# pvangoor/eqvio

Measured on AMD Instinct MI355X. Metric: EqF vision updates/sec @ N=200 landmarks, higher is better.
Workload: dtype f64; 1 GPU; synthetic 'hover' world, 200 tracked landmarks (state dim 621, 400 measurement rows), InvDepth chart, fast Riccati, IMU 200 Hz / camera 20 Hz (10 observer steps per frame), EuRoC pinhole intrinsics, one independent filter per GPU (replicas); landmarks=200, state_dim=621, parallelism=replicas x1

## Files before the change

eqvio_amd/capi.py:

```python
import ctypes as C
import os

import numpy as np

_HERE = os.path.dirname(os.path.abspath(__file__))
LIB_DIR = os.environ.get("EQVIO_AMD_LIB_DIR") or os.path.join(_HERE, "lib")

COORD_EUCLIDEAN, COORD_INVDEPTH, COORD_NORMAL = 0, 1, 2
OPT_RICCATI_DENSE, OPT_CHECK_FINITE, OPT_SIGMA_FP32, OPT_DOORBELL, OPT_SPECULATIVE, OPT_EARLY_LIFT, OPT_TRACE, OPT_FUSED_ASSEMBLY, OPT_LOOKAHEAD, OPT_LA_TIMEOUT_US, OPT_Z_IN_LOOKAHEAD, OPT_LA_SPLIT_ROWS, OPT_MEASURE_IN_PROPAGATE, OPT_LIFT_WITH_SYRK, OPT_LA_HOME, OPT_TILES_PER_WORKGROUP, OPT_GATHER_IN_PROPAGATE, OPT_HOLD_NEW_LANDMARKS, OPT_SELECT_ONE_WORKGROUP, OPT_LIVE_COLUMNS_FIRST, OPT_EARLY_DOORBELL, OPT_QUIET_DOOR_WAIT, OPT_INNOVATION_STATS, OPT_TIMING = 1, 2, 3, 6, 7, 8, 9, 11, 12, 15, 17, 18, 19, 20, 21, 22, 23, 24, 25, 26, 27, 29, 30, 100

c_double_p = C.POINTER(C.c_double)
c_int_p = C.POINTER(C.c_int)


class Camera(C.Structure):

    _fields_ = [
        ("model", C.c_int),
        ("width", C.c_int),
        ("height", C.c_int),
        ("fx", C.c_double),
        ("fy", C.c_double),
        ("cx", C.c_double),
        ("cy", C.c_double),
        ("dist", C.c_double * 5),
    ]

    @staticmethod
    def pinhole(fx, fy, cx, cy, width, height):
        cam = Camera()
        cam.model, cam.width, cam.height = 0, int(width), int(height)
        cam.fx, cam.fy, cam.cx, cam.cy = fx, fy, cx, cy
        return cam

    @staticmethod
    def radtan(fx, fy, cx, cy, width, height, k1, k2, p1, p2, k3=0.0):
        cam = Camera.pinhole(fx, fy, cx, cy, width, height)
        cam.model = 1
        cam.dist[:] = [k1, k2, p1, p2, k3]
        return cam

    @staticmethod
# ... 141 lines not shown
        "eqf_add_landmarks_held": (C.c_int, [vp, c_int_p, c_double_p, C.c_int, C.c_double]),
        "eqf_hold_supported": (C.c_int, [vp]),
        "eqf_hold_stats": (C.c_int, [vp, C.POINTER(C.c_long), C.c_int]),
        "eqf_live_columns_stats": (C.c_int, [vp, C.POINTER(C.c_long), C.c_int]),
        "eqf_own_hardware_queue": (C.c_int, [vp]),
        "eqf_remove_invalid_landmarks": (C.c_int, [vp]),
        "eqf_integrate_riccati_fast": (C.c_int, [vp, c_double_p, C.c_double, c_double_p, c_double_p]),
        "eqf_integrate_riccati_accurate": (C.c_int, [vp, c_double_p, C.c_double, c_double_p, c_double_p]),
        "eqf_integrate_riccati_discrete": (C.c_int, [vp, c_double_p, C.c_double, c_double_p, c_double_p]),
        "eqf_integrate_observer": (C.c_int, [vp, c_double_p, c_double_p, C.c_int, C.c_int]),
        "eqf_outlier_stats": (C.c_int, [vp, P(Camera), c_int_p, c_double_p, C.c_int, c_double_p, c_double_p, c_double_p]),
        "eqf_propagate_fast": (C.c_int, [vp, c_double_p, C.c_double, c_double_p, c_double_p, c_double_p, c_double_p, C.c_int, C.c_int]),
        "eqf_stage_measurement": (C.c_int, [vp, c_int_p, c_double_p, C.c_int]),
        "eqf_trace_read": (C.c_int, [vp, C.POINTER(C.c_ulonglong), C.POINTER(C.c_longlong), C.POINTER(C.c_uint)]),
        "eqf_host_wait_stats": (C.c_int, [vp, C.POINTER(C.c_long), c_double_p, C.c_int]),
        "eqf_stats_then_update": (C.c_int, [vp, C.POINTER(Camera), c_int_p, c_double_p, C.c_int, C.c_double, C.c_double, C.c_double, C.c_int, C.c_int, c_double_p, c_double_p,
                                  c_double_p, c_int_p]),
        "eqf_stats_select_update": (C.c_int, [vp, C.POINTER(Camera), c_int_p, c_double_p, C.c_int, C.c_double, C.c_double, C.c_int, C.c_double, C.c_int, C.c_int, c_double_p,
                                    c_double_p, c_double_p, c_int_p, c_int_p, c_int_p]),
        "eqf_vision_update": (C.c_int, [vp, P(Camera), c_int_p, c_double_p, C.c_int, C.c_double, C.c_int, C.c_int]),
        "eqf_last_gamma": (C.c_int, [vp, c_double_p, C.c_int]),
        "eqf_compute_nees": (C.c_int, [vp, c_double_p, c_int_p, c_double_p, C.c_int, c_double_p]),
        "eqf_nees_lu_fallbacks": (C.c_int, [vp, C.POINTER(C.c_long)]),
        "eqf_speculation_stats": (C.c_int, [vp, C.POINTER(C.c_long), C.POINTER(C.c_long), C.POINTER(C.c_long), C.c_int]),
        "eqf_measure_in_propagate_stats": (C.c_int, [vp, C.POINTER(C.c_long), C.c_int]),
        "eqf_z_in_lookahead_stats": (C.c_int, [vp, C.POINTER(C.c_long), C.c_int]),
        "eqf_gather_stats": (C.c_int, [vp, C.POINTER(C.c_long), C.c_int]),
        "eqf_selection_stats": (C.c_int, [vp, C.POINTER(C.c_long), C.POINTER(C.c_long), C.c_int]),
        "eqf_output_cov_all": (C.c_int, [vp, P(Camera), c_double_p]),
        "eqf_lookahead_stats": (C.c_int, [vp, C.POINTER(C.c_long), C.POINTER(C.c_long), C.c_int]),
        "eqf_debug_matrices_AB": (C.c_int, [vp, c_double_p, c_double_p, c_double_p]),
        "eqf_debug_get_W": (C.c_int, [vp, c_double_p, C.c_int, C.c_int]),
        "eqf_debug_syrk_order": (C.c_int, [C.c_int, c_int_p]),
        "eqf_debug_lookahead_stamps": (C.c_int, [vp, C.POINTER(C.c_ulonglong)]),
        "eqf_debug_matrix_C": (C.c_int, [vp, P(Camera), c_int_p, c_double_p, C.c_int, C.c_int, c_double_p, c_double_p]),
        "eqf_mfma_f64_peak": (C.c_int, [vp, c_double_p]),
        "eqf_mfma_f64_peak_clock": (C.c_int, [vp, C.POINTER(C.c_double), C.POINTER(C.c_double)]),
        "eqf_last_kernel_times": (C.c_int, [vp, c_int_p, P(C.c_float), C.c_int]),
        "eqf_last_innovation": (C.c_int, [vp, c_int_p, c_double_p, c_double_p]),
        "eqf_innovation_totals": (C.c_int, [vp, P(C.c_long), P(C.c_long), c_double_p, c_double_p]),
        "eqf_reset_innovation_totals": (C.c_int, [vp]),
    }
    for name, (res, args) in protos.items():
        if os.environ.get("EQVIO_AMD_LIB_DIR") and name in ("eqf_lookahead_home", "eqf_device_to_itself", "eqf_early_doorbell_stats", "eqf_update_unsettled", "eqf_remove_invalid_at_update", "eqf_gather_stats", "eqf_remove_unmeasured_landmarks", "eqf_find_unknown_ids", "eqf_add_landmarks_held", "eqf_hold_supported", "eqf_hold_stats", "eqf_same_as_mapped", "eqf_live_columns_stats", "eqf_own_hardware_queue", "eqf_last_innovation", "eqf_innovation_totals", "eqf_reset_innovation_totals") and not hasattr(lib, name):
            continue
        fn = getattr(lib, name)
        fn.restype = res
        fn.argtypes = args
    lib._declared = sorted(protos)
    _lib = lib
    return lib


class EqfCore:

    def __init__(self, max_landmarks, coordinate_choice=COORD_EUCLIDEAN, device=0):
        self.lib = load_eqf_lib()
        self.h = C.c_void_p()
        self._chk0(self.lib.eqf_create(C.byref(self.h), device, max_landmarks, coordinate_choice))
        self._cap0 = max_landmarks + 16

    def _chk0(self, rc):
        if rc != 0:
            raise EqfError(rc, self.lib.eqf_error_string(rc).decode())

    def close(self):
        if self.h:
            self.lib.eqf_destroy(self.h)
            self.h = C.c_void_p()

    def __del__(self):
        try:
            self.close()
        except Exception:
            pass

    @property
# ... 557 lines not shown
```

eqvio_amd/csrc/eqf_hip.hip:

```cpp
#include "eqf_hip.h"
#include "eqf_kernels.hpp"
#include "eqf_lookahead.hpp"
#include "eqf_innovation.hpp"
#include "eqf_batch.hpp"
#include "eqf_batch.h"
#include "host_prof.hpp"
#include <algorithm>
#include <atomic>
#include <chrono>
#include <condition_variable>
#include <deque>
#include <limits>
#include <mutex>
#include <optional>
#include <cstdio>
#include <cstdlib>
#include <cstring>
#include <string>
#include <vector>
#include <unistd.h>
#include <fcntl.h>
#include <signal.h>
#include <sys/mman.h>
#include <cerrno>
// ... 69 lines not shown
    g.bacc = v3(s[3], s[4], s[5]);
    g.A = Pose{Qt{s[6], s[7], s[8], s[9]}, v3(s[10], s[11], s[12])};
    g.w = v3(s[13], s[14], s[15]);
    g.B = Pose{Qt{s[16], s[17], s[18], s[19]}, v3(s[20], s[21], s[22])};
    return g;
}
void pack_group(const GroupSensor& g, double* s) {
    pack_v3(g.bgyr, s);
    pack_v3(g.bacc, s + 3);
    pack_pose(g.A, s + 6, s + 10);
    pack_v3(g.w, s + 13);
    pack_pose(g.B, s + 16, s + 20);
}

}

struct TailPlan {
    int M = 0, m = 0, n = 0, rows = 0;
    double meas_var = 0.0;
    int discreteCorr = 0;
    const int* spec = nullptr;
    int spec_seq = 0;
    bool use_door = false;
    int door_seq = 0;
    MeasFuse mf{};
    const int* live_cols = nullptr;
    bool ident = false;
    bool la = false;
    bool chain_only = false;
    int zb = 0;
    bool build_z = false;
    bool in_prop = false;
    bool lift_with_syrk = false;
    bool lift_before_syrk = false;
    bool syrk_gamma = false;
    int early_seq = 0;
    bool sig32 = false, check = false;
    bool innov = false;
    bool masked = false;
};


struct CtxOptions {
    int opt_dense = 0, opt_check = 0, opt_timing = 0, opt_f32 = 0, opt_early = 1, opt_fuse_asm = 1;
    int opt_door = 1;
    int opt_spec = 1;
    int opt_la_home = 1;
    int opt_lookahead = 1;
    int opt_zb = 1;
    int opt_zb_large = 1;
    int opt_la_split = 1;
    int opt_prop_tpw = 1;
    int opt_gather = 1;
    int opt_early_door = 1;
    int opt_quiet_wait = 1;
    int opt_la_watch_ahead = 1;
    int opt_hold = 1;
    int opt_sel_one = 1;
    int opt_live_first = 1;
    int opt_measure_prop = 1;
    int opt_lift_syrk = 1;
    int opt_innov = 0;
    long long la_timeout_ticks = LA_TIMEOUT_TICKS;
};
struct CtxCounters {
    long la_launches = 0, la_fallbacks = 0;
    int la_consecutive_stalls = 0;
    long la_home_launches = 0;
    long la_home_refused = 0;
    long la_book_timeouts = 0;
    long zb_launches = 0;
    long early_rings = 0;
    long live_first_launches = 0;
    long held_launches = 0;
    long gather_launches = 0;
    long me_used = 0;
    int spec_backoff = 0, spec_backoff_len = 0;
    long spec_calls = 0, spec_queued = 0, spec_cancelled = 0;
    long sel_frames = 0, sel_discarded = 0;
    long nees_lu_fallbacks = 0;
    long wait_calls = 0, launch_calls = 0;
    double wait_seconds = 0.0, launch_seconds = 0.0;
    long innov_updates = 0, innov_dof = 0;
    double innov_nis = 0.0, innov_logdet = 0.0;
    int innov_last_kind = 0;
    int innov_last_dof = 0;
    double innov_last_nis = 0.0, innov_last_logdet = 0.0;
};
enum { INNOV_NONE = 0, INNOV_VALUE, INNOV_FAILED, INNOV_OFF };
struct InnovPending {
    int kind, slot, seq, m;
};
struct CtxBuffers {
    std::vector<void*> device, pinned;
};

struct eqf_ctx : CtxOptions, CtxCounters {
    CtxBuffers own;
    int device = 0;
    hipStream_t stream = nullptr;
    hipStream_t stream2 = nullptr;
    hipEvent_t ev_assembled = nullptr, ev_observer = nullptr, ev_early = nullptr;
    bool ev_assembled_early = false;
    bool obs_pending = false;
    bool busy_common = false, busy_steps = false, busy_meas = false;
    int chart = 0;
    int Ncap = 0, ncap = 0, ld = 0;
    int mcap = 0, ldz = 0;
    int N = 0;
// ... 840 lines not shown
    return 0;
}

enum OptKind { OPT_PLAIN, OPT_BOOL , OPT_RANGE  };
struct OptRow {
    int id;
    int CtxOptions::*member;
    OptKind kind;
    int lo, hi;
};
static const OptRow kOptions[] = {
    {EQF_OPT_RICCATI_DENSE, &CtxOptions::opt_dense, OPT_PLAIN, 0, 0},
    {EQF_OPT_CHECK_FINITE, &CtxOptions::opt_check, OPT_PLAIN, 0, 0},
    {EQF_OPT_SIGMA_FP32, &CtxOptions::opt_f32, OPT_RANGE, 0, 3},
    {EQF_OPT_SPECULATIVE, &CtxOptions::opt_spec, OPT_PLAIN, 0, 0},
    {EQF_OPT_DOORBELL, &CtxOptions::opt_door, OPT_PLAIN, 0, 0},
    {EQF_OPT_EARLY_LIFT, &CtxOptions::opt_early, OPT_PLAIN, 0, 0},
    {EQF_OPT_FUSED_ASSEMBLY, &CtxOptions::opt_fuse_asm, OPT_PLAIN, 0, 0},
    {EQF_OPT_LOOKAHEAD, &CtxOptions::opt_lookahead, OPT_PLAIN, 0, 0},
    {EQF_OPT_LA_TIMEOUT_US, nullptr, OPT_RANGE, 0, INT_MAX},
    {EQF_OPT_Z_IN_LOOKAHEAD, nullptr, OPT_PLAIN, 0, 0},
    {EQF_OPT_LA_SPLIT_ROWS, &CtxOptions::opt_la_split, OPT_BOOL, 0, 0},
    {EQF_OPT_LA_HOME, &CtxOptions::opt_la_home, OPT_PLAIN, 0, 0},
    {EQF_OPT_TILES_PER_WORKGROUP, &CtxOptions::opt_prop_tpw, OPT_RANGE, 0, 8},
    {EQF_OPT_GATHER_IN_PROPAGATE, &CtxOptions::opt_gather, OPT_BOOL, 0, 0},
    {EQF_OPT_HOLD_NEW_LANDMARKS, &CtxOptions::opt_hold, OPT_BOOL, 0, 0},
    {EQF_OPT_SELECT_ONE_WORKGROUP, &CtxOptions::opt_sel_one, OPT_BOOL, 0, 0},
    {EQF_OPT_LIVE_COLUMNS_FIRST, &CtxOptions::opt_live_first, OPT_BOOL, 0, 0},
    {EQF_OPT_EARLY_DOORBELL, &CtxOptions::opt_early_door, OPT_BOOL, 0, 0},
    {EQF_OPT_QUIET_DOOR_WAIT, &CtxOptions::opt_quiet_wait, OPT_BOOL, 0, 0},
    {EQF_OPT_MEASURE_IN_PROPAGATE, &CtxOptions::opt_measure_prop, OPT_BOOL, 0, 0},
    {EQF_OPT_LIFT_WITH_SYRK, &CtxOptions::opt_lift_syrk, OPT_BOOL, 0, 0},
    {EQF_OPT_INNOVATION_STATS, &CtxOptions::opt_innov, OPT_BOOL, 0, 0},
    {EQF_OPT_TRACE, nullptr, OPT_PLAIN, 0, 0},
    {100, &CtxOptions::opt_timing, OPT_PLAIN, 0, 0},
    {102, &CtxOptions::opt_la_watch_ahead, OPT_BOOL, 0, 0},
};
static const OptRow* option_row(int option) {
    for (const OptRow& r : kOptions)
        if (r.id == option)
            return &r;
    return nullptr;
}

int eqf_get_option(const eqf_ctx* c, int option, int* value) {
    const OptRow* row = c && value ? option_row(option) : nullptr;
    if (!row)
        return EQF_E_BAD_ARG;
    if (row->member)
        *value = c->*(row->member);
    else if (option == EQF_OPT_Z_IN_LOOKAHEAD)
        *value = c->opt_zb ? (c->opt_zb_large ? 1 : 2) : 0;
    else if (option == EQF_OPT_LA_TIMEOUT_US)
        *value = (int)(c->la_timeout_ticks / 100);
    else
        *value = c->d_trace ? 1 : 0;
    return 0;
}
int eqf_set_option(eqf_ctx* c, int option, int value) {
    const OptRow* row = c ? option_row(option) : nullptr;
    if (!row)
        return EQF_E_BAD_ARG;
    if (row->kind == OPT_BOOL)
        value = value ? 1 : 0;
    else if (row->kind == OPT_RANGE && (value < row->lo || value > row->hi))
        return EQF_E_BAD_ARG;
// ... 1545 lines not shown
    c->la_home_force = true;
    int rc = lookahead_selftest_pass(c, refused);
    c->la_home_force = false;
    if (rc)
        return rc;
    const bool home_on = c->opt_la_home != 0;
    if (home_on && (refused || c->la_selftest < 0)) {
        std::fprintf(stderr, "[eqf_hip] device %d: the look-ahead kernel's HOME placement %s; this context uses the classic placement\n", c->device,
                     refused ? "was refused (blocks are not dealt to the XCDs round robin)" : "failed its self-test");
        c->opt_la_home = 0;
        c->la_selftest = 0;
        rc = lookahead_selftest_pass(c, refused);
        if (rc)
            return rc;
    }
    if (c->la_selftest < 0)
        std::fprintf(stderr, "[eqf_hip] look-ahead self-test failed on device %d: this context factorises on the launch chain\n", c->device);
    c->la_home_launches = 0;
    return 0;
}
static bool tail_use_door(const eqf_ctx* c) { return c->opt_door && !c->opt_check && !c->obs_pending; }
struct TailCall {
    const int* ids;
    int M;
    double meas_var;
    int discreteCorr;
    bool use_door;
    int door_seq;
    const MeasFuse* fuse = nullptr;
    bool live_first = false;
    bool takes_early = false;
    bool masked = false;
};
static void plan_tail(const eqf_ctx* c, TailPlan& p, const TailCall& call, bool chain_only) {
    const int M = call.M;
    const MeasFuse* fuse = call.fuse;
    p = TailPlan{};
    p.M = M, p.m = 2 * M, p.n = c->n(), p.rows = p.m + p.n + 1;
    p.meas_var = call.meas_var, p.discreteCorr = call.discreteCorr, p.use_door = call.use_door, p.door_seq = call.door_seq;
    if (fuse)
        p.mf = *fuse, p.spec = fuse->spec_w, p.spec_seq = fuse->spec_seq;
    p.sig32 = c->sig32, p.check = c->opt_check != 0;
    p.innov = c->opt_innov != 0 && c->d_Linv_all && c->h_innov, p.masked = call.masked;
    const int NJ = blocks(p.m, 32);
    p.ident = !call.live_first && c->map_ident && c->map_gen == c->lm_gen && c->map_N == c->N && (int)c->map_ids.size() == M && std::equal(call.ids, call.ids + M, c->map_ids.begin());
    p.live_cols = (call.live_first && NJ <= 16) ? c->d_spec + 2 : nullptr;
    const bool eligible = lookahead_eligible(c, p.m);
    p.chain_only = chain_only, p.la = eligible && !chain_only;
    const bool zb_ok = c->opt_zb && !c->sig32 && !chain_only && eligible && (NJ <= 16 || c->opt_zb_large);
    p.in_prop = fuse && c->me_valid && c->opt_measure_prop && fuse->y == c->d_meas && c->opt_early && c->me_M == M && c->me_gen == c->lm_gen && c->me_star == fuse->star &&
                same_cam(c->me_cam, fuse->cam) && !c->sig32;
    p.zb = !zb_ok ? 0 : (!fuse ? 1 : (p.in_prop ? 3 : ((fuse->y == c->d_meas && c->opt_early && NJ <= 8) ? 2 : 0)));
    p.build_z = p.zb == 0;
    const bool lift_can_ride = c->opt_early && c->opt_lift_syrk && !c->sig32 && c->opt_timing != 1;
    const bool early_door_ok = lift_can_ride && !c->opt_check;
    p.lift_with_syrk = lift_can_ride && c->N > 0;
    p.lift_before_syrk = c->opt_early != 0;
    p.syrk_gamma = !(p.lift_before_syrk || p.la);
    p.early_seq = (p.la && call.use_door && call.takes_early && c->opt_early_door && early_door_ok) ? call.door_seq : 0;
}
static TailPlan retry_plan(const TailPlan& stalled, bool use_door, int door_seq) {
    TailPlan p = stalled;
    p.use_door = use_door, p.door_seq = door_seq;
    p.spec = nullptr, p.spec_seq = 0, p.mf = MeasFuse{};
    p.live_cols = nullptr;
    p.la = false, p.chain_only = true, p.early_seq = 0;
    p.build_z = stalled.zb != 0, p.zb = 0, p.in_prop = false;
    p.syrk_gamma = !p.lift_before_syrk;
    return p;
}
static LiftArgs lift_args(eqf_ctx* c, const TailPlan& p, const double* gpart, int stall_seq) {
    return LiftArgs{c->N, c->Ncap, c->chart, p.discreteCorr, c->d_gamma, c->q0(), c->Qq(), c->Qa(), c->h_res + 3 * (size_t)c->Ncap, c->h_res + 7 * (size_t)c->Ncap, c->d_flags,
                    c->h_resflags, p.use_door ? c->d_door + 1 : nullptr, c->h_door + 1, p.door_seq, p.spec, p.spec_seq, gpart, c->ld, trace_slot(c, TR_LIFT), stall_seq};
}
static int launch_lift(eqf_ctx* c, const TailPlan& p, const double* gpart, int stall_seq) {
    KTimer t(c, KN_LIFT);
    hipLaunchKernelGGL(k_lift, dim3(blocks(c->N, 64)), dim3(64), 0, c->stream, lift_args(c, p, gpart, stall_seq));
    HIPCHK(hipGetLastError());
    return 0;
}
static int launch_build_Z(eqf_ctx* c, const TailPlan& p) {
    KTimer t(c, KN_BUILD_Z);
    const bool fused = p.mf.enabled != 0;
    auto launch = [&](auto kern, auto* sig) {
        hipLaunchKernelGGL(kern, dim3(blocks(p.n + p.M + 1, 256), blocks(p.M, BZ_JB) + 1 + (fused ? 1 : 0)), dim3(256), 0, c->stream, p.n, p.M, c->Ncap, c->ld, c->ldz, p.meas_var, c->d_lmidx, sig,
                           c->d_C, c->d_ytil, c->d_Z, linv_base(c, p), c->d_flags, fused ? (const int*)nullptr : p.spec, p.spec_seq, p.mf, trace_slot(c, TR_BUILD_Z));
    };
    if (p.in_prop)
        launch(k_build_Z<double, true, true>, (const double*)c->sigma());
// ... 63 lines not shown
            break;
        }
    if (++c->innov_seq <= 0)
        c->innov_seq = 1;
    c->innov_cur_slot = slot, c->innov_cur_seq = c->innov_seq;
    InnovArgs a{};
    a.m = p.m, a.rows = p.rows, a.ldz = c->ldz;
    a.W = c->d_W;
    a.tiles = p.la ? c->d_pub : c->d_Linv_all;
    a.lmidx = c->d_lmidx, a.removed = p.masked ? c->h_sel : nullptr, a.nlm = c->N;
    a.spec = p.spec, a.spec_seq = p.spec_seq;
    a.flags = c->d_flags, a.stall_seq = stall_seq;
    a.out = c->h_innov + slot, a.seq = c->innov_seq;
    KTimer t(c, KN_INNOVATION);
    launch_innovation_kernel(a, c->stream);
    HIPCHK(hipGetLastError());
    return 0;
}
static int launch_tail(eqf_ctx* c, const TailPlan& p) {
    LaBookingGuard booking{c};
    if (p.in_prop)
        ++c->me_used;
    if (p.build_z)
        EQFCHK(launch_build_Z(c, p));
    host_stamp(c, TH_BUILD_Z_OUT);
    if (p.la) {
        ++c->la_launches;
        EQFCHK(launch_lookahead(c, p));
    } else
        EQFCHK(launch_chain(c, p.rows, p.m, c->ldz, c->d_Z, c->d_W, true, p.spec, p.spec_seq, p.lift_before_syrk ? c->d_gpart : nullptr, p.innov ? c->d_Linv_all : nullptr));
    const int stall_seq = p.la ? c->la_seq : -1;
    const double* gpart = p.la ? nullptr : c->d_gpart;
    const int nt = blocks(p.n, 32);
    if (p.lift_with_syrk) {
        const int nlift = blocks(c->N, 64);
        KTimer t(c, KN_SYRK);
        hipLaunchKernelGGL(HIP_KERNEL_NAME(k_syrk_lift<double>), dim3(nlift + nt * (nt + 1) / 2), dim3(64 * SYRK_NW), 0, c->stream, p.n, p.m, c->ld, c->ldz, c->d_W, (double*)c->sigma(),
                           c->d_gamma, c->d_flags, trace_slot(c, TR_SYRK), c->d_syrk_order + c->syrk_off[nt], lift_args(c, p, gpart, stall_seq), nlift, p.live_cols, nt <= SYRK_ARITH_TILES ? nt : 0);
        HIPCHK(hipGetLastError());
    } else {
        if (p.lift_before_syrk)
            EQFCHK(launch_lift(c, p, gpart, stall_seq));
        KTimer t(c, KN_SYRK);
        auto launch = [&](auto kern, auto* sig) {
            hipLaunchKernelGGL(kern, dim3(nt * (nt + 1) / 2), dim3(64 * SYRK_NW), 0, c->stream, p.n, p.m, c->ld, c->ldz, c->d_W, sig, nt, c->d_gamma, p.spec, p.spec_seq, p.syrk_gamma ? 1 : 0, c->d_flags,
                               trace_slot(c, TR_SYRK), c->d_syrk_order + c->syrk_off[nt], stall_seq);
        };
        if (p.sig32 && p.syrk_gamma)
            launch(k_syrk_sub<float, true>, (float*)c->sigma());
        else if (p.sig32)
            launch(k_syrk_sub<float, false>, (float*)c->sigma());
        else if (p.syrk_gamma)
            launch(k_syrk_sub<double, true>, (double*)c->sigma());
        else
            launch(k_syrk_sub<double, false>, (double*)c->sigma());
        HIPCHK(hipGetLastError());
    }
    EQFCHK(round_sigma(c, p.spec, p.spec_seq));
    if (!p.lift_with_syrk && !p.lift_before_syrk)
        EQFCHK(launch_lift(c, p, nullptr, stall_seq));
    if (p.check)
        EQFCHK(launch_check_finite(c));
    if (p.innov)
        EQFCHK(launch_innovation(c, p, stall_seq));
    booking.keep = p.la;
    return 0;
}
// ... 491 lines not shown
    return 0;
}
int eqf_z_in_lookahead_stats(eqf_ctx* c, long* launches, int reset) {
    if (!c || !launches)
        return EQF_E_BAD_ARG;
    *launches = c->zb_launches;
    if (reset)
        c->zb_launches = 0;
    return 0;
}
int eqf_gather_stats(eqf_ctx* c, long* launches, int reset) {
    if (!c || !launches)
        return EQF_E_BAD_ARG;
    *launches = c->gather_launches;
    if (reset)
        c->gather_launches = 0;
    return 0;
}
int eqf_speculation_stats(eqf_ctx* c, long* calls, long* queued, long* cancelled, int reset) {
    if (!c || !calls || !queued || !cancelled)
        return EQF_E_BAD_ARG;
    *calls = c->spec_calls;
    *queued = c->spec_queued;
    *cancelled = c->spec_cancelled;
    if (reset)
        c->spec_calls = c->spec_queued = c->spec_cancelled = 0;
    return 0;
}

int eqf_debug_syrk_order(int nt, int* tile_of_block) {
    if (nt < 1 || nt > 4095 || !tile_of_block)
        return EQF_E_BAD_ARG;
    build_syrk_order(nt, tile_of_block);
    return 0;
}
int eqf_lookahead_stats(eqf_ctx* c, long* launches, long* fallbacks, int reset) {
    if (!c)
        return EQF_E_BAD_ARG;
    if (launches)
        *launches = c->la_launches;
    if (fallbacks)
        *fallbacks = c->la_fallbacks;
    if (reset)
        c->la_launches = c->la_fallbacks = 0;
    return 0;
}

int eqf_lookahead_selftest(const eqf_ctx* c) { return c ? c->la_selftest : EQF_E_BAD_ARG; }
int eqf_lookahead_home(const eqf_ctx* c, int* home_xcd, long* home_launches) {
    if (!c)
        return EQF_E_BAD_ARG;
    if (home_xcd)
        *home_xcd = (c->opt_la_home && c->cu_count == 256) ? c->la_home : -1;
    if (home_launches)
        *home_launches = c->la_home_launches;
    return 0;
}

int eqf_early_doorbell_stats(eqf_ctx* c, long* updates, int reset) {
    if (!c)
        return EQF_E_BAD_ARG;
    if (updates)
        *updates = c->early_rings;
    if (reset)
        c->early_rings = 0;
    return 0;
// ... 282 lines not shown
```

eqvio_amd/csrc/eqf_kernels.hpp:

```cpp
#pragma once
#include "eqf_math.hpp"
#include "eqvio_types.h"
#include <hip/hip_runtime.h>

namespace eqf {

struct Common {
    double Mv[9];
    double RTic[9];
    double RTicSx[9];
    double CT[36];
    double vC[3];
    double Ass[441];
    double Bs[252];
};
struct CommonK {
    double lm[66];
    double RA[9];
    double SxRA[9];
    double RAsv[9];
    double G[9];
    double adT[36];
};
constexpr int kObsChunk = 20;
// ... 2068 lines not shown
    const double g0 = gamma_row(gamma, gpart, ldg, 21 + 3 * ic), g1 = gamma_row(gamma, gpart, ldg, 21 + 3 * ic + 1), g2 = gamma_row(gamma, gpart, ldg, 21 + 3 * ic + 2);
    const LiftIn in = lift_load(ic, Ncap, chart, discrete, q0, Qq, Qa);
    const int f0 = flags[0], f1 = flags[1], f3 = flags[3] == stall_seq ? 1 : 0;
    const int specv = spec ? __hip_atomic_load(spec, __ATOMIC_RELAXED, __HIP_MEMORY_SCOPE_AGENT) : 0;
    const bool aborted = spec && specv == spec_seq;
    const bool failed = f0 != 0 || f3 != 0;
    if (i == 0) {
        flags_host[2] = aborted ? 1 : 0;
        flags_host[3] = f3;
    }
    if (!aborted && i == 0) {
        flags_host[0] = f0;
        flags_host[1] = f1;
    }
    if (!aborted && !failed) {
        if (i < 21) {
            gamma_host[i] = gs;
            if (gpart)
                gamma[i] = gs;
        }
        if (lm) {
            if (gpart) {
                gamma[21 + 3 * i] = g0;
                gamma[21 + 3 * i + 1] = g1;
                gamma[21 + 3 * i + 2] = g2;
            }
            lift_landmark(i, V3{g0, g1, g2}, in, N, Ncap, chart, discrete, Qq, Qa, est);
        }
    }
    ring_doorbell(la.door_count, la.door_host, la.door_seq, nblk);
    trace_end(tr);
}
__global__ void __launch_bounds__(64) k_lift(const LiftArgs la) { lift_block(la, (int)blockIdx.x, (int)gridDim.x); }
template <typename TS>
__global__ void __launch_bounds__(64 * SYRK_NW) k_syrk_lift(int n, int m, int ld, int ldz, const double* __restrict__ Wb, TS* __restrict__ Sig, double* __restrict__ gamma,
                                                            const int* __restrict__ flags, trace_t* tr, const int* __restrict__ tile_of_block, const LiftArgs la, int nlift, const int* __restrict__ live_cols, int nt_arith) {
    if ((int)blockIdx.x < nlift) {
        if (threadIdx.x < 64)
            lift_block(la, (int)blockIdx.x, nlift);
        return;
    }
    syrk_sub_tile<TS, false>(n, m, ld, ldz, Wb, Sig, gamma, la.spec, la.spec_seq, flags, tr, tile_of_block, la.stall_seq, (int)blockIdx.x - nlift, live_cols, nt_arith);
}
__global__ void __launch_bounds__(64) k_estimate(int N, int Ncap, const double* __restrict__ q0, const double* __restrict__ Qq, const double* __restrict__ Qa,
                                                 double* __restrict__ est, int* __restrict__ door_count = nullptr, int* __restrict__ door_host = nullptr, int door_seq = 0) {
    const int i = blockIdx.x * blockDim.x + threadIdx.x;
    if (i < N) {
        const double a = Qa[i];
        const V3 qh = (1.0 / a) * q_rot(q_inv(ldq(Qq, Ncap, i)), ld3(q0, Ncap, i));
        est[i] = qh.x;
        est[N + i] = qh.y;
        est[2 * N + i] = qh.z;
        est[3 * N + i] = (a <= 1e-8 || a > 1e8 || !(a == a)) ? 1.0 : 0.0;
    }
    ring_doorbell(door_count, door_host, door_seq);
}

__global__ void k_scatter_landmarks(int k, int dst0, int Ncap, const double* __restrict__ p_aos, const double* __restrict__ Q_aos, double* __restrict__ q0,
                                    double* __restrict__ Qq, double* __restrict__ Qa) {
    const int t = blockIdx.x * blockDim.x + threadIdx.x;
    if (t >= k)
        return;
    const int i = dst0 + t;
    for (int c = 0; c < 3; ++c)
        q0[c * Ncap + i] = p_aos[3 * t + c];
    {
        const V3 p{p_aos[3 * t], p_aos[3 * t + 1], p_aos[3 * t + 2]};
        double* cc = q0 + (size_t)CC_OFF * Ncap;
        store_chart_constants(cc, Ncap, i, p.x, p.y, p.z, nullptr);
    }
    if (Q_aos) {
        for (int c = 0; c < 4; ++c)
            Qq[c * Ncap + i] = Q_aos[5 * t + c];
        Qa[i] = Q_aos[5 * t + 4];
    } else {
// ... 769 lines not shown
```

include/eqf_hip.h:

```cpp
#ifndef EQF_HIP_H
#define EQF_HIP_H
#include "eqvio_types.h"

#ifdef __cplusplus
extern "C" {
#endif

typedef struct eqf_ctx eqf_ctx;

enum {
    EQF_OK = 0,
    EQF_E_NONFINITE = -1,
    EQF_E_NOT_SPD = -2,
    EQF_E_BAD_ARG = -3,
    EQF_E_CAPACITY = -4,
    EQF_E_NO_DEVICE = -5,
    EQF_E_UNSUPPORTED = -6,
    EQF_E_STALLED = -7
};

enum {
    EQF_OPT_RICCATI_DENSE = 1,
    EQF_OPT_CHECK_FINITE = 2,
    EQF_OPT_SPECULATIVE = 7,
    EQF_OPT_DOORBELL = 6,
    EQF_OPT_EARLY_LIFT = 8,
    EQF_OPT_TRACE = 9,
    EQF_OPT_FUSED_ASSEMBLY = 11,
    EQF_OPT_LOOKAHEAD = 12,
    EQF_OPT_LA_TIMEOUT_US = 15,
    EQF_OPT_Z_IN_LOOKAHEAD = 17,
    EQF_OPT_LA_SPLIT_ROWS = 18,
    EQF_OPT_MEASURE_IN_PROPAGATE = 19,
    EQF_OPT_LIFT_WITH_SYRK = 20,
    EQF_OPT_LA_HOME = 21,
    EQF_OPT_TILES_PER_WORKGROUP = 22,
    EQF_OPT_GATHER_IN_PROPAGATE = 23,
    EQF_OPT_HOLD_NEW_LANDMARKS = 24,
    EQF_OPT_EARLY_DOORBELL = 27,
    EQF_OPT_QUIET_DOOR_WAIT = 29,
    EQF_OPT_SELECT_ONE_WORKGROUP = 25,
    EQF_OPT_LIVE_COLUMNS_FIRST = 26,
    EQF_OPT_INNOVATION_STATS = 30,
    EQF_OPT_SIGMA_FP32 = 3
};

const char* eqf_error_string(int code);

int eqf_create(eqf_ctx** out, int device, int max_landmarks, int coordinate_choice);
void eqf_destroy(eqf_ctx* ctx);
int eqf_set_option(eqf_ctx* ctx, int option, int value);
int eqf_get_option(const eqf_ctx* ctx, int option, int* value);
int eqf_synchronize(eqf_ctx* ctx);
int eqf_num_landmarks(const eqf_ctx* ctx);
int eqf_get_ids(const eqf_ctx* ctx, int* ids, int cap);
void* eqf_stream(eqf_ctx* ctx);

int eqf_set_state(eqf_ctx* ctx, const double* xi0_sensor, const double* X_sensor, const int* ids, const double* q0, const double* Q, int N);
int eqf_get_state(eqf_ctx* ctx, double* xi0_sensor, double* X_sensor, int* ids, double* q0, double* Q, int cap);

int eqf_set_sigma(eqf_ctx* ctx, const double* sigma_colmajor, int n);
int eqf_set_sigma_diag(eqf_ctx* ctx, const double* diag, int n);
int eqf_get_sigma(eqf_ctx* ctx, double* sigma_colmajor, int n);
int eqf_get_sigma_block(eqf_ctx* ctx, int r0, int c0, int rows, int cols, double* out_colmajor);

int eqf_state_estimate(eqf_ctx* ctx, double* sensor, int* ids, double* p, int cap);

int eqf_add_landmarks(eqf_ctx* ctx, const int* ids, const double* p, int k, double var);
int eqf_add_landmarks_held(eqf_ctx* ctx, const int* ids, const double* p, int k, double var);
int eqf_hold_supported(const eqf_ctx* ctx);
int eqf_hold_stats(eqf_ctx* ctx, long* launches, int reset);
int eqf_remove_landmarks(eqf_ctx* ctx, const int* indices, int k);
int eqf_remove_unmeasured_landmarks(eqf_ctx* ctx, const int* ids, int M, int* removed_idx, int* n_removed);
int eqf_find_unknown_ids(eqf_ctx* ctx, const int* ids, int M, int* unknown_j, int* n_unknown);
int eqf_same_as_mapped(const eqf_ctx* ctx, const int* ids, int M);
int eqf_remove_invalid_landmarks(eqf_ctx* ctx);
// ... 10 lines not shown
int eqf_output_cov_all(eqf_ctx* ctx, const eqvio_camera* cam, double* out4N);

int eqf_vision_update(eqf_ctx* ctx, const eqvio_camera* cam, const int* ids, const double* y, int M, double meas_var, int useEquivariantOutput, int discreteCorrection);

int eqf_propagate_fast(eqf_ctx* ctx, const double* imu13_mean, double dt_total, const double* Qdiag12, const double* Pdiag8, const double* imu13_k, const double* dt_k,
                       int k, int discreteLift);
int eqf_stage_measurement(eqf_ctx* ctx, const int* ids, const double* y_px, int M);

int eqf_stats_then_update(eqf_ctx* ctx, const eqvio_camera* cam, const int* ids, const double* y_px, int M, double thrAbs, double thrProb, double meas_var,
                          int useEquivariantOutput, int discreteCorrection, double* absErr, double* probErr, double* depth2, int* updated);

int eqf_speculation_stats(eqf_ctx* ctx, long* calls, long* queued, long* cancelled, int reset);
int eqf_measure_in_propagate_stats(eqf_ctx* ctx, long* used, int reset);
int eqf_z_in_lookahead_stats(eqf_ctx* ctx, long* launches, int reset);
int eqf_gather_stats(eqf_ctx* ctx, long* launches, int reset);
int eqf_stats_select_update(eqf_ctx* ctx, const eqvio_camera* cam, const int* ids, const double* y_px, int M, double thrAbs, double thrProb, int max_outliers, double meas_var,
                            int useEquivariantOutput, int discreteCorrection, double* absErr, double* probErr, double* depth2, int* updated, int* removed_idx, int* n_removed);
int eqf_lookahead_stats(eqf_ctx* ctx, long* launches, long* fallbacks, int reset);
int eqf_own_hardware_queue(eqf_ctx* ctx);
int eqf_live_columns_stats(eqf_ctx* ctx, long* launches, int reset);
int eqf_lookahead_selftest(const eqf_ctx* ctx);
int eqf_lookahead_home(const eqf_ctx* ctx, int* home_xcd, long* home_launches);
int eqf_device_to_itself(eqf_ctx* ctx);
int eqf_selection_stats(eqf_ctx* ctx, long* frames, long* discarded, int reset);

int eqf_last_gamma(eqf_ctx* ctx, double* out, int cap);

int eqf_compute_nees(eqf_ctx* ctx, const double* true_sensor, const int* true_ids, const double* true_p, int n_true, double* nees);
int eqf_nees_lu_fallbacks(eqf_ctx* ctx, long* count);

int eqf_debug_matrices_AB(eqf_ctx* ctx, const double* imu13, double* A_out, double* B_out);
int eqf_debug_get_W(eqf_ctx* ctx, double* out, int rows, int cols);
int eqf_debug_syrk_order(int nt, int* tile_of_block);
int eqf_debug_matrix_C(eqf_ctx* ctx, const eqvio_camera* cam, const int* ids, const double* y, int M, int useEquivariantOutput, double* C_out, double* ytilde_out);

int eqf_mfma_f64_peak(eqf_ctx* ctx, double* tflops);
int eqf_mfma_f64_peak_clock(eqf_ctx* ctx, double* tflops, double* sclk_ghz);

int eqf_last_innovation(eqf_ctx* ctx, int* dof, double* nis, double* logdet);
int eqf_innovation_totals(eqf_ctx* ctx, long* updates, long* dof, double* nis, double* logdet);
int eqf_reset_innovation_totals(eqf_ctx* ctx);
int eqf_last_kernel_times(eqf_ctx* ctx, int* which, float* usec, int cap);
int eqf_trace_read(eqf_ctx* ctx, unsigned long long* device_ticks, long long* host_ns, unsigned* last_frame);
int eqf_debug_lookahead_stamps(eqf_ctx* ctx, unsigned long long* out768);
int eqf_host_wait_stats(eqf_ctx* ctx, long* calls, double* seconds, int reset);
const char* eqf_kernel_name(int which);

#ifdef __cplusplus
}
#endif
#endif
```

Baseline: 11570 updates/s.

## Add one-round SYRK with one workgroup per tile when the grid fits the CUs

Adds a SYRK path used when the lift blocks plus one workgroup per lower-triangular 32x32 tile fit in a single wave of CUs. Each workgroup covers the whole K range of its tile. Its waves stride over K, prefetch deep register batches of W into fp64 MFMAs, then reduce the partial sums through a swizzled LDS buffer and write both triangles of Sigma. This replaces the sub-tiled SYRK scheduling and is meant to cut the latency of this step on the Riccati update path. The cost is more LDS and registers per workgroup, and a different reduction order.

```diff
diff --git a/eqvio_amd/capi.py b/eqvio_amd/capi.py
--- a/eqvio_amd/capi.py
+++ b/eqvio_amd/capi.py
@@ -7,7 +7,7 @@
 LIB_DIR = os.environ.get("EQVIO_AMD_LIB_DIR") or os.path.join(_HERE, "lib")
 
 COORD_EUCLIDEAN, COORD_INVDEPTH, COORD_NORMAL = 0, 1, 2
-OPT_RICCATI_DENSE, OPT_CHECK_FINITE, OPT_SIGMA_FP32, OPT_DOORBELL, OPT_SPECULATIVE, OPT_EARLY_LIFT, OPT_TRACE, OPT_FUSED_ASSEMBLY, OPT_LOOKAHEAD, OPT_LA_TIMEOUT_US, OPT_Z_IN_LOOKAHEAD, OPT_LA_SPLIT_ROWS, OPT_MEASURE_IN_PROPAGATE, OPT_LIFT_WITH_SYRK, OPT_LA_HOME, OPT_TILES_PER_WORKGROUP, OPT_GATHER_IN_PROPAGATE, OPT_HOLD_NEW_LANDMARKS, OPT_SELECT_ONE_WORKGROUP, OPT_LIVE_COLUMNS_FIRST, OPT_EARLY_DOORBELL, OPT_QUIET_DOOR_WAIT, OPT_INNOVATION_STATS, OPT_TIMING = 1, 2, 3, 6, 7, 8, 9, 11, 12, 15, 17, 18, 19, 20, 21, 22, 23, 24, 25, 26, 27, 29, 30, 100
+OPT_RICCATI_DENSE, OPT_CHECK_FINITE, OPT_SIGMA_FP32, OPT_DOORBELL, OPT_SPECULATIVE, OPT_EARLY_LIFT, OPT_TRACE, OPT_FUSED_ASSEMBLY, OPT_LOOKAHEAD, OPT_LA_TIMEOUT_US, OPT_Z_IN_LOOKAHEAD, OPT_LA_SPLIT_ROWS, OPT_MEASURE_IN_PROPAGATE, OPT_LIFT_WITH_SYRK, OPT_LA_HOME, OPT_TILES_PER_WORKGROUP, OPT_GATHER_IN_PROPAGATE, OPT_HOLD_NEW_LANDMARKS, OPT_SELECT_ONE_WORKGROUP, OPT_LIVE_COLUMNS_FIRST, OPT_EARLY_DOORBELL, OPT_QUIET_DOOR_WAIT, OPT_INNOVATION_STATS, OPT_SYRK_ONE_ROUND, OPT_TIMING = 1, 2, 3, 6, 7, 8, 9, 11, 12, 15, 17, 18, 19, 20, 21, 22, 23, 24, 25, 26, 27, 29, 30, 31, 100
 
 c_double_p = C.POINTER(C.c_double)
 c_int_p = C.POINTER(C.c_int)
@@ -215,6 +215,8 @@
         "eqf_debug_matrices_AB": (C.c_int, [vp, c_double_p, c_double_p, c_double_p]),
         "eqf_debug_get_W": (C.c_int, [vp, c_double_p, C.c_int, C.c_int]),
         "eqf_debug_syrk_order": (C.c_int, [C.c_int, c_int_p]),
+        "eqf_debug_syrk_one_round": (C.c_int, [C.c_int, C.c_int, C.c_int]),
+        "eqf_syrk_one_round_stats": (C.c_int, [vp, C.POINTER(C.c_long), C.c_int]),
         "eqf_debug_lookahead_stamps": (C.c_int, [vp, C.POINTER(C.c_ulonglong)]),
         "eqf_debug_matrix_C": (C.c_int, [vp, P(Camera), c_int_p, c_double_p, C.c_int, C.c_int, c_double_p, c_double_p]),
         "eqf_mfma_f64_peak": (C.c_int, [vp, c_double_p]),
@@ -225,7 +227,7 @@
         "eqf_reset_innovation_totals": (C.c_int, [vp]),
     }
     for name, (res, args) in protos.items():
-        if os.environ.get("EQVIO_AMD_LIB_DIR") and name in ("eqf_lookahead_home", "eqf_device_to_itself", "eqf_early_doorbell_stats", "eqf_update_unsettled", "eqf_remove_invalid_at_update", "eqf_gather_stats", "eqf_remove_unmeasured_landmarks", "eqf_find_unknown_ids", "eqf_add_landmarks_held", "eqf_hold_supported", "eqf_hold_stats", "eqf_same_as_mapped", "eqf_live_columns_stats", "eqf_own_hardware_queue", "eqf_last_innovation", "eqf_innovation_totals", "eqf_reset_innovation_totals") and not hasattr(lib, name):
+        if os.environ.get("EQVIO_AMD_LIB_DIR") and name in ("eqf_lookahead_home", "eqf_device_to_itself", "eqf_early_doorbell_stats", "eqf_update_unsettled", "eqf_remove_invalid_at_update", "eqf_gather_stats", "eqf_remove_unmeasured_landmarks", "eqf_find_unknown_ids", "eqf_add_landmarks_held", "eqf_hold_supported", "eqf_hold_stats", "eqf_same_as_mapped", "eqf_live_columns_stats", "eqf_own_hardware_queue", "eqf_last_innovation", "eqf_innovation_totals", "eqf_reset_innovation_totals", "eqf_debug_syrk_one_round", "eqf_syrk_one_round_stats") and not hasattr(lib, name):
             continue
         fn = getattr(lib, name)
         fn.restype = res
diff --git a/eqvio_amd/csrc/eqf_hip.hip b/eqvio_amd/csrc/eqf_hip.hip
--- a/eqvio_amd/csrc/eqf_hip.hip
+++ b/eqvio_amd/csrc/eqf_hip.hip
@@ -125,6 +125,7 @@
     bool build_z = false;
     bool in_prop = false;
     bool lift_with_syrk = false;
+    bool syrk_one_round = false;
     bool lift_before_syrk = false;
     bool syrk_gamma = false;
     int early_seq = 0;
@@ -154,6 +155,7 @@
     int opt_measure_prop = 1;
     int opt_lift_syrk = 1;
     int opt_innov = 0;
+    int opt_syrk_one_round = 1;
     long long la_timeout_ticks = LA_TIMEOUT_TICKS;
 };
 struct CtxCounters {
@@ -168,6 +170,7 @@
     long held_launches = 0;
     long gather_launches = 0;
     long me_used = 0;
+    long syrk_one_round_launches = 0;
     int spec_backoff = 0, spec_backoff_len = 0;
     long spec_calls = 0, spec_queued = 0, spec_cancelled = 0;
     long sel_frames = 0, sel_discarded = 0;
@@ -1074,6 +1077,7 @@
     {EQF_OPT_MEASURE_IN_PROPAGATE, &CtxOptions::opt_measure_prop, OPT_BOOL, 0, 0},
     {EQF_OPT_LIFT_WITH_SYRK, &CtxOptions::opt_lift_syrk, OPT_BOOL, 0, 0},
     {EQF_OPT_INNOVATION_STATS, &CtxOptions::opt_innov, OPT_BOOL, 0, 0},
+    {EQF_OPT_SYRK_ONE_ROUND, &CtxOptions::opt_syrk_one_round, OPT_BOOL, 0, 0},
     {EQF_OPT_TRACE, nullptr, OPT_PLAIN, 0, 0},
     {100, &CtxOptions::opt_timing, OPT_PLAIN, 0, 0},
     {102, &CtxOptions::opt_la_watch_ahead, OPT_BOOL, 0, 0},
@@ -2685,6 +2689,10 @@
     bool takes_early = false;
     bool masked = false;
 };
+static bool syrk_one_round_fits(int N, int cu_count) {
+    const int nt = blocks(21 + 3 * N, 32);
+    return N > 0 && blocks(N, 64) + nt * (nt + 1) / 2 <= cu_count;
+}
 static void plan_tail(const eqf_ctx* c, TailPlan& p, const TailCall& call, bool chain_only) {
     const int M = call.M;
     const MeasFuse* fuse = call.fuse;
@@ -2708,6 +2716,7 @@
     const bool lift_can_ride = c->opt_early && c->opt_lift_syrk && !c->sig32 && c->opt_timing != 1;
     const bool early_door_ok = lift_can_ride && !c->opt_check;
     p.lift_with_syrk = lift_can_ride && c->N > 0;
+    p.syrk_one_round = p.lift_with_syrk && c->opt_syrk_one_round && syrk_one_round_fits(c->N, c->cu_count);
     p.lift_before_syrk = c->opt_early != 0;
     p.syrk_gamma = !(p.lift_before_syrk || p.la);
     p.early_seq = (p.la && call.use_door && call.takes_early && c->opt_early_door && early_door_ok) ? call.door_seq : 0;
@@ -2837,7 +2846,14 @@
     const int stall_seq = p.la ? c->la_seq : -1;
     const double* gpart = p.la ? nullptr : c->d_gpart;
     const int nt = blocks(p.n, 32);
-    if (p.lift_with_syrk) {
+    if (p.syrk_one_round) {
+        const int nlift = blocks(c->N, 64);
+        ++c->syrk_one_round_launches;
+        KTimer t(c, KN_SYRK);
+        hipLaunchKernelGGL(HIP_KERNEL_NAME(k_syrk_lift<double, true>), dim3(nlift + nt * (nt + 1) / 2), dim3(64 * SYRK_NW), 0, c->stream, p.n, p.m, c->ld, c->ldz, c->d_W, (double*)c->sigma(),
+                           c->d_gamma, c->d_flags, trace_slot(c, TR_SYRK), (const int*)nullptr, lift_args(c, p, gpart, stall_seq), nlift, p.live_cols, 0);
+        HIPCHK(hipGetLastError());
+    } else if (p.lift_with_syrk) {
         const int nlift = blocks(c->N, 64);
         KTimer t(c, KN_SYRK);
         hipLaunchKernelGGL(HIP_KERNEL_NAME(k_syrk_lift<double>), dim3(nlift + nt * (nt + 1) / 2), dim3(64 * SYRK_NW), 0, c->stream, p.n, p.m, c->ld, c->ldz, c->d_W, (double*)c->sigma(),
@@ -3395,6 +3411,16 @@
     if (nt < 1 || nt > 4095 || !tile_of_block)
         return EQF_E_BAD_ARG;
     build_syrk_order(nt, tile_of_block);
+    return 0;
+}
+int eqf_debug_syrk_one_round(int N, int cu_count, int lift_rides) { return lift_rides && syrk_one_round_fits(N, cu_count) ? 1 : 0; }
+int eqf_syrk_one_round_stats(eqf_ctx* c, long* launches, int reset) {
+    if (!c)
+        return EQF_E_BAD_ARG;
+    if (launches)
+        *launches = c->syrk_one_round_launches;
+    if (reset)
+        c->syrk_one_round_launches = 0;
     return 0;
 }
 int eqf_lookahead_stats(eqf_ctx* c, long* launches, long* fallbacks, int reset) {
diff --git a/eqvio_amd/csrc/eqf_kernels.hpp b/eqvio_amd/csrc/eqf_kernels.hpp
--- a/eqvio_amd/csrc/eqf_kernels.hpp
+++ b/eqvio_amd/csrc/eqf_kernels.hpp
@@ -2124,7 +2124,113 @@
     trace_end(tr);
 }
 __global__ void __launch_bounds__(64) k_lift(const LiftArgs la) { lift_block(la, (int)blockIdx.x, (int)gridDim.x); }
-template <typename TS>
+
+constexpr int SYRK_OR_DEPTH = 13;
+__device__ __forceinline__ int syrk_or_pos(int i, int j) { return 32 * j + (i ^ j); }
+template <int D>
+__device__ __forceinline__ void syrk_tile_one_round(double* __restrict__ sred , int n, int m, int ld, int ldz, const double* __restrict__ Wb, double* __restrict__ Sig, const int* __restrict__ spec, int spec_seq,
+                                                    const int* __restrict__ flags, trace_t* tr, int stall_seq, int blk, const int* __restrict__ live_cols) {
+    constexpr int NW = SYRK_NW;
+    int bi = (int)((sqrtf(8.0f * (float)blk + 1.0f) - 1.0f) * 0.5f);
+    while ((bi + 1) * (bi + 2) / 2 <= blk)
+        ++bi;
+    while (bi * (bi + 1) / 2 > blk)
+        --bi;
+    const int bj = blk - bi * (bi + 1) / 2;
+    const int i0 = bi * 32, j0 = bj * 32;
+    const double* W = Wb + m;
+    const int tid = threadIdx.x;
+    const int wave = __builtin_amdgcn_readfirstlane(tid >> 6), lane = tid & 63;
+    const int lr = lane & 15, lk = lane >> 4;
+    const int ia = min(i0 + lr, n - 1), ib = min(i0 + 16 + lr, n - 1);
+    const int ja = min(j0 + lr, n - 1), jb = min(j0 + 16 + lr, n - 1);
+    const double zia = (i0 + lr < n) ? 1.0 : 0.0, zib = (i0 + 16 + lr < n) ? 1.0 : 0.0;
+    const double zja = (j0 + lr < n) ? 1.0 : 0.0, zjb = (j0 + 16 + lr < n) ? 1.0 : 0.0;
+    d4 acc00 = {0, 0, 0, 0}, acc10 = acc00, acc01 = acc00, acc11 = acc00;
+    double pa[D], pb[D], qa[D], qb[D];
+    auto request = [&](int s0) {
+#pragma unroll
+        for (int s = 0; s < D; ++s) {
+            const size_t kc = (size_t)min(4 * (s0 + NW * s) + lk, m - 1);
+            pa[s] = W[ia + kc * ldz];
+            pb[s] = W[ib + kc * ldz];
+            qa[s] = W[ja + kc * ldz];
+            qb[s] = W[jb + kc * ldz];
+        }
+    };
+    auto multiply = [&](int s0, int nsteps) {
+#pragma unroll
+        for (int s = 0; s < D; ++s) {
+            const int st = s0 + NW * s;
+            if (st < nsteps) {
+                const double zk = 4 * st + lk < m ? 1.0 : 0.0;
+                const double a = pa[s] * (zia * zk), b = pb[s] * (zib * zk);
+                const double qa_ = qa[s] * zja, qb_ = qb[s] * zjb;
+                acc00 = __builtin_amdgcn_mfma_f64_16x16x4f64(qa_, a, acc00, 0, 0, 0);
+                acc10 = __builtin_amdgcn_mfma_f64_16x16x4f64(qa_, b, acc10, 0, 0, 0);
+                acc01 = __builtin_amdgcn_mfma_f64_16x16x4f64(qb_, a, acc01, 0, 0, 0);
+                acc11 = __builtin_amdgcn_mfma_f64_16x16x4f64(qb_, b, acc11, 0, 0, 0);
+            }
+        }
+    };
+    const int live_raw = live_cols ? __hip_atomic_load(live_cols, __ATOMIC_RELAXED, __HIP_MEMORY_SCOPE_AGENT) : 0;
+    request(wave);
+    const int ti = tid & 31, tj = tid >> 5;
+    const int i = i0 + ti;
+    double sig_pre[2];
+#pragma unroll
+    for (int e = 0; e < 2; ++e) {
+        const int j = j0 + tj + 16 * e;
+        sig_pre[e] = (i < n && j < n && (bi != bj || i >= j)) ? Sig[i + (size_t)j * ld] : 0.0;
+    }
+    const int f0 = __hip_atomic_load(flags, __ATOMIC_RELAXED, __HIP_MEMORY_SCOPE_AGENT), f3 = __hip_atomic_load(flags + 3, __ATOMIC_RELAXED, __HIP_MEMORY_SCOPE_AGENT);
+    const int specv = spec ? __hip_atomic_load(spec, __ATOMIC_RELAXED, __HIP_MEMORY_SCOPE_AGENT) : 0;
+    const int mk = live_cols ? min(m, 32 * max((__builtin_amdgcn_readfirstlane(live_raw) + 31) >> 5, 1)) : m;
+    const int nsteps = (mk + 3) >> 2;
+    multiply(wave, nsteps);
+    for (int s0 = wave + NW * D; s0 < nsteps; s0 += NW * D) {
+        request(s0);
+        multiply(s0, nsteps);
+    }
+    {
+        double* mine = sred + wave * 1024;
+#pragma unroll
+        for (int r = 0; r < 4; ++r) {
+            const int j = lk + 4 * r;
+            mine[syrk_or_pos(lr, j)] = acc00[r];
+            mine[syrk_or_pos(16 + lr, j)] = acc10[r];
+            mine[syrk_or_pos(lr, 16 + j)] = acc01[r];
+            mine[syrk_or_pos(16 + lr, 16 + j)] = acc11[r];
+        }
+    }
+    __syncthreads();
+    if (spec && specv == spec_seq)
+        return;
+    if (f0 | (f3 == stall_seq ? 1 : 0))
+        return;
+#pragma unroll
+    for (int e = 0; e < 2; ++e) {
+        const int tje = tj + 16 * e, j = j0 + tje;
+        const int idx = syrk_or_pos(ti, tje);
+        double t = 0.0;
+        t += (sred[idx] + sred[1024 + idx]) + (sred[2048 + idx] + sred[3072 + idx]);
+        t += (sred[4096 + idx] + sred[5120 + idx]) + (sred[6144 + idx] + sred[7168 + idx]);
+        const double v = sig_pre[e] - t;
+        if (i < n && j < n && (bi != bj || i >= j))
+            Sig[i + (size_t)j * ld] = v;
+        sred[idx] = v;
+    }
+    __syncthreads();
+    const int mj = j0 + ti;
+#pragma unroll
+    for (int e = 0; e < 2; ++e) {
+        const int tie = tj + 16 * e, mi = i0 + tie;
+        if (mi < n && mj < n && (bi != bj || tie > ti))
+            Sig[mj + (size_t)mi * ld] = sred[syrk_or_pos(tie, ti)];
+    }
+    trace_end(tr);
+}
+template <typename TS, bool ONE_ROUND = false>
 __global__ void __launch_bounds__(64 * SYRK_NW) k_syrk_lift(int n, int m, int ld, int ldz, const double* __restrict__ Wb, TS* __restrict__ Sig, double* __restrict__ gamma,
                                                             const int* __restrict__ flags, trace_t* tr, const int* __restrict__ tile_of_block, const LiftArgs la, int nlift, const int* __restrict__ live_cols, int nt_arith) {
     if ((int)blockIdx.x < nlift) {
@@ -2132,7 +2238,22 @@
             lift_block(la, (int)blockIdx.x, nlift);
         return;
     }
-    syrk_sub_tile<TS, false>(n, m, ld, ldz, Wb, Sig, gamma, la.spec, la.spec_seq, flags, tr, tile_of_block, la.stall_seq, (int)blockIdx.x - nlift, live_cols, nt_arith);
+    if constexpr (!ONE_ROUND) {
+        syrk_sub_tile<TS, false>(n, m, ld, ldz, Wb, Sig, gamma, la.spec, la.spec_seq, flags, tr, tile_of_block, la.stall_seq, (int)blockIdx.x - nlift, live_cols, nt_arith);
+    } else {
+        static_assert(sizeof(TS) == sizeof(double), "the one-round form is for the fp64 store");
+        __shared__ double sred[1024 * SYRK_NW];
+        const int blk = (int)blockIdx.x - nlift;
+        if (tr && blk == 0 && threadIdx.x == 0)
+            *tr = wall_clock64();
+        const int nreq = (m + 3) >> 2;
+        if (nreq <= 4 * SYRK_NW)
+            syrk_tile_one_round<4>(sred, n, m, ld, ldz, Wb, Sig, la.spec, la.spec_seq, flags, tr, la.stall_seq, blk, live_cols);
+        else if (nreq <= 7 * SYRK_NW)
+            syrk_tile_one_round<7>(sred, n, m, ld, ldz, Wb, Sig, la.spec, la.spec_seq, flags, tr, la.stall_seq, blk, live_cols);
+        else
+            syrk_tile_one_round<SYRK_OR_DEPTH>(sred, n, m, ld, ldz, Wb, Sig, la.spec, la.spec_seq, flags, tr, la.stall_seq, blk, live_cols);
+    }
 }
 __global__ void __launch_bounds__(64) k_estimate(int N, int Ncap, const double* __restrict__ q0, const double* __restrict__ Qq, const double* __restrict__ Qa,
                                                  double* __restrict__ est, int* __restrict__ door_count = nullptr, int* __restrict__ door_host = nullptr, int door_seq = 0) {
diff --git a/include/eqf_hip.h b/include/eqf_hip.h
--- a/include/eqf_hip.h
+++ b/include/eqf_hip.h
@@ -42,6 +42,7 @@
     EQF_OPT_SELECT_ONE_WORKGROUP = 25,
     EQF_OPT_LIVE_COLUMNS_FIRST = 26,
     EQF_OPT_INNOVATION_STATS = 30,
+    EQF_OPT_SYRK_ONE_ROUND = 31,
     EQF_OPT_SIGMA_FP32 = 3
 };
 
@@ -118,6 +119,8 @@
 int eqf_debug_matrices_AB(eqf_ctx* ctx, const double* imu13, double* A_out, double* B_out);
 int eqf_debug_get_W(eqf_ctx* ctx, double* out, int rows, int cols);
 int eqf_debug_syrk_order(int nt, int* tile_of_block);
+int eqf_debug_syrk_one_round(int N, int cu_count, int lift_rides);
+int eqf_syrk_one_round_stats(eqf_ctx* ctx, long* launches, int reset);
 int eqf_debug_matrix_C(eqf_ctx* ctx, const eqvio_camera* cam, const int* ids, const double* y, int M, int useEquivariantOutput, double* C_out, double* ytilde_out);
 
 int eqf_mfma_f64_peak(eqf_ctx* ctx, double* tflops);
```

After: 11630 updates/s, median of 6. No clear change (+0.4%).
